# balkce/beamform

Hardware: AMD Instinct MI355X
Metric: stft_frames_per_sec (higher is better)
Workload: dtype f64; 1 GPU; das 8-mic 1024-pt (hop 512), 65536-frame batch per GPU, 1 stream(s), planar input resident in HBM; frames_per_gpu=65536, frames_fed_per_gpu=65536, mics=8, fft=1024, hop=512, streams=1, layout=planar, gather=n/a, parallelism=independent batches x1, input=uniform noise in [-0.5, 0.5), settle_launches_before_warmup=408, forward_transforms_per_frame_pair=6

## Files before the change

### beamform_amd/csrc/das_f64_plan.hpp

```cpp
#pragma once

#include <cstdlib>
#include <cstring>

#if defined(__HIPCC__)
#define BF_PLAN_HD __host__ __device__ inline
#else
#define BF_PLAN_HD inline
#endif

namespace bf {

constexpr int kChunkEnd = 0xFFFFF;
constexpr int kMaxChunkPairs = 1000;
constexpr int kSchedMaxChunks = 16384;

struct DasSchedPlan {
    int n_levels;
    int cnt[8], size[8];
    int n_chunks;
    int grid;
};

BF_PLAN_HD void das_f64_chunk(const DasSchedPlan &p, long n_frames, int n_streams, int k, int *stream, long *t0, long *n) {
    int lvl = 0, kk = k;
    long pair0 = 0;
    while (lvl < p.n_levels - 1 && kk >= p.cnt[lvl] * n_streams) {
        kk -= p.cnt[lvl] * n_streams;
        pair0 += (long)p.cnt[lvl] * p.size[lvl];
        ++lvl;
    }
    const int s = kk / p.cnt[lvl], j = kk - s * p.cnt[lvl];
    *stream = s;
    *t0 = 2 * (pair0 + (long)j * p.size[lvl]);
    long len = 2L * p.size[lvl];
    if (*t0 + len > n_frames) len = n_frames - *t0;
    *n = len;
}

inline DasSchedPlan das_f64_plan(long n_frames, int n_streams, int n_cus, const char *env) {
    DasSchedPlan p{};
    const long pairs = (n_frames + 1) / 2;
    long nb = (long)n_cus / n_streams;
    if (nb < 1) nb = 1;
    int sizes[8], n_sizes = 0;
    const long share = (pairs + nb - 1) / nb;
    if (env && strchr(env, ',')) {
        const char *c = env;
        while (*c && n_sizes < 8) {
            sizes[n_sizes++] = atoi(c);
            c = strchr(c, ',');
            if (!c) break;
            ++c;
        }
    } else if (!(env && atoi(env) == 0) && share >= 48) {
        long front = (share * 13 / 16) & ~7L;
        long rest = share - front;
        while (front > kMaxChunkPairs && n_sizes < 3) {
            sizes[n_sizes++] = kMaxChunkPairs;
            front -= kMaxChunkPairs;
        }
        if (front > kMaxChunkPairs) { rest += front - kMaxChunkPairs; front = kMaxChunkPairs; }
        sizes[n_sizes++] = (int)front;
        while (n_sizes < 6 && rest >= 24) {
            long sz = (rest / 2) & ~7L;
            if (sz > kMaxChunkPairs) sz = kMaxChunkPairs;
            sizes[n_sizes++] = (int)sz;
            rest -= sz;
        }
        if (rest >= 12) { sizes[n_sizes++] = 4; rest -= 4; }
        sizes[n_sizes++] = 2;
// ... 33 lines not shown
```

### beamform_amd/csrc/das_f64_w64.hip

```cpp
#include <hip/hip_runtime.h>

#include <type_traits>

#include "launch_trace.hpp"
#include "pipeline_kernels.hpp"
#include "switches.hpp"
#include "w64_f64_dev.hpp"

namespace bf {

namespace {

constexpr int kBlock = 512;
constexpr int kWaves = kBlock / 64;
constexpr int kHop = 512;
constexpr int kTwD = 2 * (1024 + 4 * kTw2RowW64Rot);
constexpr int oTw = 0;
constexpr int oPlane = kTwD;
constexpr int oGain = oPlane + kWaves * kPlaneD;
constexpr int oCross = oGain + 4 * 2048;
constexpr int oFlag = oCross + 512;
constexpr int kWinRow = 18;
constexpr int oWin = oFlag + 8;
constexpr int kLdsD = oWin + 64 * kWinRow;
// ... 253 lines not shown
constexpr int kGMic = 8 * kGRow;
constexpr int kSlots = 64;
constexpr int kTwP = 2 * (960 + 4 * kTw2RowW64Rot);
constexpr int pTw = 0;
constexpr int pPlane = kTwP;
constexpr int pGain = pPlane + kWaves * kPlaneD;
constexpr int pFlag = pGain + 7 * kGMic * 2;
constexpr int kRingR = 32;
constexpr int kRingSlots = kRingR + kWaves;
constexpr int pRing = pFlag + (kSlots + 4) / 2;
constexpr int pWin = pRing + kRingR / 2;
constexpr int kLdsP = pWin + 64 * kWinRow;
static_assert(kLdsP * 8 <= 160 * 1024, "LDS");
static_assert((pGain & 1) == 0 && (pWin & 1) == 0, "16-byte alignment");


typedef volatile __attribute__((address_space(3))) int *lds_int_t;
typedef volatile __attribute__((address_space(3))) unsigned long long *lds_u64_t;
__device__ __forceinline__ int lds_fetch_add(lds_int_t p, int v, int lane) {
    int old = 0;
    if (lane == 0) old = __hip_atomic_fetch_add((__attribute__((address_space(3))) int *)p, v, __ATOMIC_RELAXED, __HIP_MEMORY_SCOPE_WORKGROUP);
    return __builtin_amdgcn_readfirstlane(old);
}
__device__ __forceinline__ unsigned long long lds_fetch_add64(lds_u64_t p, int lane) {
    unsigned long long old = 0;
    if (lane == 0) old = __hip_atomic_fetch_add((__attribute__((address_space(3))) unsigned long long *)p, 1ull, __ATOMIC_RELAXED, __HIP_MEMORY_SCOPE_WORKGROUP);
    const unsigned lo = (unsigned)__builtin_amdgcn_readfirstlane((int)(unsigned)old), hi = (unsigned)__builtin_amdgcn_readfirstlane((int)(unsigned)(old >> 32));
    return ((unsigned long long)hi << 32) | lo;
}
struct DasSched {
    const int4 *chunks;
    unsigned *counter;
    int n_chunks;
};
__device__ __forceinline__ unsigned long long pack_work(unsigned vbase, int chunk, int pairs, int next) {
    return ((unsigned long long)(vbase & 0xFFFFFFu) << 40) | ((unsigned long long)(unsigned)chunk << 20) | ((unsigned long long)(unsigned)pairs << 10) | (unsigned)next;
}
struct PairWork {
    int4 d;
    int pos;
    int len;
    unsigned u;
    bool have;
};
__device__ __forceinline__ int4 load_chunk(const int4 *chunks, int k) {
    const int4 d = chunks[k];
    return int4{__builtin_amdgcn_readfirstlane(d.x), __builtin_amdgcn_readfirstlane(d.y), __builtin_amdgcn_readfirstlane(d.z), k};
}
__device__ __forceinline__ PairWork draw_pair(lds_u64_t work, const DasSched &sc, int lane, const int4 held) {
    PairWork r;
    r.have = false;
    r.d = int4{0, 0, 0, 0};
    r.pos = r.len = 0;
    r.u = 0;
    for (;;) {
        const unsigned long long old = lds_fetch_add64(work, lane);
        const int pos = (int)(old & 1023u), len = (int)((old >> 10) & 1023u), k = (int)((old >> 20) & 0xFFFFFu);
        const unsigned vb = (unsigned)(old >> 40);
        if (k == kChunkEnd) return r;
        if (pos < len) {
            if (k == held.w) r.d = held;
            else r.d = load_chunk(sc.chunks, k);
            r.pos = pos; r.len = len; r.u = vb + (unsigned)pos; r.have = true;
            return r;
        }
        if (pos == len) {
            unsigned k2 = 0;
            if (lane == 0) k2 = __hip_atomic_fetch_add(sc.counter, 1u, __ATOMIC_RELAXED, __HIP_MEMORY_SCOPE_AGENT);
            k2 = (unsigned)__builtin_amdgcn_readfirstlane((int)k2);
            if (k2 >= (unsigned)sc.n_chunks) {
                if (lane == 0) *work = pack_work(vb + (unsigned)len, kChunkEnd, 0, 0);
                return r;
            }
            r.d = load_chunk(sc.chunks, (int)k2);
            r.len = (r.d.z + 1) >> 1;
            r.pos = 0; r.u = vb + (unsigned)len; r.have = true;
            if (lane == 0) *work = pack_work(r.u, (int)k2, r.len, 1);
            return r;
        }
        while ((int)((*work >> 20) & 0xFFFFFu) == k) __builtin_amdgcn_s_sleep(2);
    }
}
__device__ __forceinline__ int claim_boundary(lds_int_t st, unsigned b, int lane) {
    const int base = 4 * (int)(b / kSlots);
    while (st[b & (kSlots - 1)] < base) __builtin_amdgcn_s_sleep(1);
    return lds_fetch_add(st + (b & (kSlots - 1)), 1, lane) - base;
}
__device__ __forceinline__ void publish_boundary(lds_int_t st, unsigned b, int lane) { (void)lds_fetch_add(st + (b & (kSlots - 1)), 2, lane); }
__device__ __forceinline__ void skip_boundary(lds_int_t st, unsigned b, int lane) {
    const int base = 4 * (int)(b / kSlots);
    while (st[b & (kSlots - 1)] < base) __builtin_amdgcn_s_sleep(1);
    (void)lds_fetch_add(st + (b & (kSlots - 1)), 4, lane);
}
__device__ __forceinline__ void await_boundary(lds_int_t st, unsigned b) {
    while (st[b & (kSlots - 1)] - 4 * (int)(b / kSlots) < 3) __builtin_amdgcn_s_sleep(1);
}

#ifdef BF_W64_STATS
__device__ unsigned long long g_stats[256 * 8 * 5];
#define BF_STATS_DECL unsigned long long st_[5] = {0, 0, 0, 0, 0}; const unsigned long long st_t0_ = __builtin_amdgcn_s_memrealtime()
#define BF_STAT(i) (++st_[i])
#define BF_STAT_WAIT_BEGIN const unsigned long long st_w0_ = __builtin_amdgcn_s_memrealtime()
#define BF_STAT_WAIT_END st_[3] += __builtin_amdgcn_s_memrealtime() - st_w0_
#define BF_STATS_FLUSH do { st_[4] = __builtin_amdgcn_s_memrealtime() - st_t0_; if (lane == 0 && blockIdx.x < 256) for (int i_ = 0; i_ < 5; ++i_) g_stats[(blockIdx.x * 8 + w) * 5 + i_] = st_[i_]; } while (0)
#else
#define BF_STATS_DECL
#define BF_STAT(i) ((void)0)
#define BF_STAT_WAIT_BEGIN
#define BF_STAT_WAIT_END
#define BF_STATS_FLUSH
#endif
#ifdef BF_W64_STAMPS
__device__ unsigned long long g_stamps[256 * 8 * 64];
#define BF_STAMP(slot) do { if (lane == 0 && blockIdx.x < 256 && (slot) < 64) g_stamps[(blockIdx.x * 8 + w) * 64 + (slot)] = __builtin_amdgcn_s_memrealtime(); } while (0)
#else
// ... 160 lines not shown
        }
        __builtin_amdgcn_fence(__ATOMIC_ACQUIRE, "workgroup");
        return r;
    };
    auto release_pair = [&](const PairWork &pw, bool has_t) {
        const unsigned u2 = 2u * pw.u;
        (void)lds_fetch_add(s_ring + (u2 & (kRingR - 1)), 2, lane);
        (void)lds_fetch_add(s_ring + ((u2 + 1) & (kRingR - 1)), has_t ? 1 : 2, lane);
        if (pw.pos > 0) (void)lds_fetch_add(s_ring + ((u2 - 1) & (kRingR - 1)), 1, lane);
    };
    auto request_ring_mic = [&](const RingHops &r, int m) { request(r.h + m * kHop, r.a + m * kHop, r.b + m * kHop); };
    auto request_ring_extra = [&](bool on, const RingHops &r) {
        if (!on) {
#pragma unroll
            for (int j = 0; j < 8; ++j) e0[j] = e1[j] = e2[j] = 0.f;
            return;
        }
#pragma unroll
        for (int j = 0; j < 8; ++j) {
            e0[j] = r.h[XM * kHop + (unsigned)(64 * j + lane)];
            e1[j] = r.a[XM * kHop + (unsigned)(64 * j + lane)];
            e2[j] = r.b[XM * kHop + (unsigned)(64 * j + lane)];
        }
    };
    RingHops curR{nullptr, nullptr, nullptr};
    (void)curR;

    BF_STAMP(0);
#ifdef BF_W64_STAMPS
    if (lane == 0 && blockIdx.x < 256) g_stamps[(blockIdx.x * 8 + w) * 64 + 59] = __builtin_amdgcn_s_memtime();
#endif
    PairWork cur;
    cur.d = load_chunk(sc.chunks, (int)blockIdx.x);
    cur.len = (cur.d.z + 1) >> 1;
    const int n_static = cur.len < kWaves ? cur.len : kWaves;
    cur.pos = w;
    cur.u = (unsigned)w;
    cur.have = w < n_static;
    if (LAYOUT == 0 && cur.have) {
        request_pair_mic(cur.d.x, cur.d.y + 2L * w, a.slot_mic[0]);
        request_extra(XM >= 0, cur.d.x, cur.d.y + 2L * w);
    } else {
        request_extra(false, 0, 0);
    }
    {
        const f64x2 *tw2 = a.tw + 64;
        f64x2 *ltw = reinterpret_cast<f64x2 *>(lds + pTw), *lg = reinterpret_cast<f64x2 *>(lds + pGain);
#pragma unroll 4
        for (int i = tid; i < kTwP / 2; i += kBlock) ltw[i] = tw2[i];
        for (int k = 0; k < NT; ++k) {
            const f64x2 *g2 = a.gains_mic + a.slot_mic[k] * kGMic;
#pragma unroll 2
            for (int i = tid; i < kGMic; i += kBlock) lg[k * kGMic + i] = g2[i];
        }
#pragma unroll 2
        for (int i = tid; i < 1024; i += kBlock) lds[pWin + (i & 63) * kWinRow + (i >> 6)] = a.win[i];
        if (tid < kSlots) s_state[tid] = 0;
        if (tid < kRingR) s_ring[tid] = 0;
        if (tid == 0) *s_work = pack_work(0u, (int)blockIdx.x, cur.len, n_static);
    }
    __syncthreads();
    BF_STAMP(1);
    BF_STATS_DECL;
    int it = 0;
    if (!cur.have) {
        cur = draw_pair(s_work, sc, lane, cur.d);
        if (LAYOUT == 0 && cur.have) {
            request_pair_mic(cur.d.x, cur.d.y + 2L * cur.pos, a.slot_mic[0]);
            request_extra(XM >= 0, cur.d.x, cur.d.y + 2L * cur.pos);
        }
    }
    while (cur.have) {
        if constexpr (LAYOUT == 1) {
            curR = prepare_pair(cur);
            request_ring_mic(curR, a.slot_mic[0]);
            request_ring_extra(XM >= 0, curR);
        }
        const int stream = cur.d.x;
        const long T0 = cur.d.y, T1 = T0 + cur.d.z;
        const long tA = T0 + 2L * cur.pos;
        const bool pair = tA + 1 < T1;
        const long tL = pair ? tA + 1 : tA;
        const unsigned u = cur.u;
        const bool has_t = cur.pos + 1 < cur.len, has_h = cur.pos > 0;
        float *ys = a.y + (long)stream * a.n_frames * kHop;
        PairWork nxt;
        nxt.have = false;
        const float *hp0 = a.x + (long)stream * a.stream_stride_x + tA * kHop;
        const float *hist0 = a.hist + (long)stream * M * kHop;
        const bool first_hop = tA < 1, last_hop = !(tA + 1 < a.n_frames);
        (void)hp0; (void)hist0; (void)first_hop; (void)last_hop;

        double Sr[16], Si[16];
        auto one_mic = [&](const int k, auto first_tag) {
            constexpr bool FIRST = decltype(first_tag)::value;
            double re[16], im[16];
#ifndef BF_PAIR_NO_VMWAIT
            if constexpr (!FIRST) __builtin_amdgcn_s_waitcnt(0x0F70);
#endif
// ... 3 lines not shown
                    const double w0 = wrow[j], w1 = wrow[j + 8];
                    const double c = (double)n1[j] + (double)e1[j];
                    const double t = ((double)n0[j] + (double)e0[j]) * w0;
                    re[j] = fma(c, w1, t);
                    re[j + 8] = fma(-c, w1, t);
                    const double t2 = c * w0, u2 = (double)n2[j] + (double)e2[j];
                    im[j] = fma(u2, w1, t2);
                    im[j + 8] = fma(-u2, w1, t2);
                }
            } else {
#pragma unroll
                for (int j = 0; j < 8; ++j) {
                    const double w0 = wrow[j], w1 = wrow[j + 8];
                    const double c = (double)n1[j];
                    const double t = (double)n0[j] * w0;
                    re[j] = fma(c, w1, t);
                    re[j + 8] = fma(-c, w1, t);
                    const double t2 = c * w0, u2 = (double)n2[j];
                    im[j] = fma(u2, w1, t2);
                    im[j + 8] = fma(-u2, w1, t2);
                }
            }
            if (__builtin_expect(!pair, 0)) {
#ifndef BF_PAIR_CNDMASK
                asm volatile("" ::: "memory");
#endif
#pragma unroll
                for (int j = 0; j < 16; ++j) im[j] = 0.0;
            }
            if (k + 1 < NT) {
                if constexpr (LAYOUT == 1) request_ring_mic(curR, a.slot_mic[k + 1]);
                else request_pair_mic(stream, tA, a.slot_mic[k + 1]);
            } else {
                nxt = draw_pair(s_work, sc, lane, cur.d);
                if constexpr (LAYOUT == 0) {
                    if (nxt.have) request_pair_mic(nxt.d.x, nxt.d.y + 2L * nxt.pos, a.slot_mic[0]);
                    else request_pair_mic(stream, tA, a.slot_mic[0]);
                }
            }
            cx<double> tw[15];
            BF_STAGE();
            load_tw1<1, 9>(tw, s_tw1, lane);
            BF_STAGE();
            fft16_core<double, -1, true, 1>(re, im);
            BF_STAGE();
            load_tw1<9, 16>(tw, s_tw1, lane);
            BF_STAGE();
            mul_tw<false, 1, 9>(re, im, tw);
            BF_STAGE();
            mul_tw<false, 9, 16>(re, im, tw);
            BF_STAGE();
            T1_fwd(re, im, wcol, row16);
            load_tw2<1, 9>(tw, s_tw2, lane);
            BF_STAGE();
            fft16_core<double, -1, true>(re, im);
            BF_STAGE();
            load_tw2<9, 16>(tw, s_tw2, lane);
            BF_STAGE();
            mul_tw<false, 1, 9>(re, im, tw);
            BF_STAGE();
            mul_tw<false, 9, 16>(re, im, tw);
            BF_STAGE();
            w64_T2_any<true>(re, im, row16 - 16 * (lane >> 4), lane >> 4);
            cxa g[16];
            const lds_gain_t gd = (lds_gain_t)(size_t)(gd0 + (unsigned)(k * kGMic * 16));
            const lds_gain_t gm = (lds_gain_t)(size_t)((g_mirror + (unsigned)(2 * k * kGMic * 16)) - (gd0 + (unsigned)(k * kGMic * 16)));
            BF_STAGE();
// ... 82 lines not shown
            oT = claim_boundary(s_state, u, lane);
            if (oT == 0) {
#pragma unroll
                for (int j = 0; j < 8; ++j) yn[(unsigned)(64 * j + lane)] = tl[j];
            }
        } else {
            skip_boundary(s_state, u, lane);
        }
#pragma unroll
        for (int j = 0; j < 16; ++j) {
            const float f = (float)Sr[j];
            oA[j] = (float)((double)f * wrow[j]);
        }
        if (pair) {
            float *y1 = ys + (tA + 1) * kHop;
#pragma unroll
            for (int j = 0; j < 8; ++j) {
                const float f0 = (float)Si[j];
                const float b0 = (float)((double)f0 * wrow[j]);
                y1[(unsigned)(64 * j + lane)] = oA[j + 8] + b0;
            }
        }
        if (has_h) {
            oH = claim_boundary(s_state, u - 1, lane);
            if (oH == 0) {
#pragma unroll
                for (int j = 0; j < 8; ++j) yo[(unsigned)(64 * j + lane)] = oA[j];
            }
        } else if (T0 == 0) {
            const float *ti = a.tail_in + (long)stream * kHop;
#pragma unroll
            for (int j = 0; j < 8; ++j) yo[(unsigned)(64 * j + lane)] = ti[(unsigned)(64 * j + lane)] + oA[j];
        } else {
#pragma unroll
            for (int j = 0; j < 8; ++j) atomicAdd(yo + (unsigned)(64 * j + lane), oA[j]);
        }
        if (oT == 0 || oH == 0) {
            __builtin_amdgcn_fence(__ATOMIC_RELEASE, "workgroup");
            if (oT == 0) publish_boundary(s_state, u, lane);
            if (oH == 0) publish_boundary(s_state, u - 1, lane);
        }
        if (oT > 0) {
            BF_STAT(2);
            BF_STAT_WAIT_BEGIN;
            await_boundary(s_state, u);
            BF_STAT_WAIT_END;
            __builtin_amdgcn_fence(__ATOMIC_ACQUIRE, "workgroup");
            float o[8];
#pragma unroll
            for (int j = 0; j < 8; ++j) o[j] = BF_PARK_LD(yn + (unsigned)(64 * j + lane));
#pragma unroll
            for (int j = 0; j < 8; ++j) yn[(unsigned)(64 * j + lane)] = tl[j] + o[j];
        } else {
            BF_STAT(0);
        }
        if (oH > 0) {
            BF_STAT(2);
            BF_STAT_WAIT_BEGIN;
            await_boundary(s_state, u - 1);
            BF_STAT_WAIT_END;
            __builtin_amdgcn_fence(__ATOMIC_ACQUIRE, "workgroup");
            float o[8];
#pragma unroll
            for (int j = 0; j < 8; ++j) o[j] = BF_PARK_LD(yo + (unsigned)(64 * j + lane));
#pragma unroll
            for (int j = 0; j < 8; ++j) yo[(unsigned)(64 * j + lane)] = o[j] + oA[j];
        } else {
            BF_STAT(1);
        }
        if (!has_t) {
            if (T1 < a.n_frames) {
                float *ynx = ys + T1 * kHop;
#pragma unroll
                for (int j = 0; j < 8; ++j) atomicAdd(ynx + (unsigned)(64 * j + lane), tl[j]);
            } else {
                float *to = a.tail_out + (long)stream * kHop;
#pragma unroll
                for (int j = 0; j < 8; ++j) to[(unsigned)(64 * j + lane)] = tl[j];
                if (a.hist_out != nullptr) {
                    float *ho = a.hist_out + (long)stream * M * kHop;
                    const float *xs = a.x + (long)stream * a.stream_stride_x;
                    for (int m = 0; m < M; ++m) {
                        const float *xl = xs + (long)m * a.mic_stride + tL * kHop;
#pragma unroll
                        for (int j = 0; j < 8; ++j) ho[m * kHop + 64 * j + lane] = xl[(unsigned)(64 * j + lane)];
                    }
                }
            }
        }
        if constexpr (LAYOUT == 1) {
            asm volatile("" ::: "memory");
            release_pair(cur, has_t);
        }
        cur = nxt;
        ++it;
    }
    BF_STATS_FLUSH;
#ifdef BF_W64_STAMPS
    if (lane == 0 && blockIdx.x < 256) {
        g_stamps[(blockIdx.x * 8 + w) * 64 + 63] = __builtin_amdgcn_s_memrealtime();
        g_stamps[(blockIdx.x * 8 + w) * 64 + 60] = __builtin_amdgcn_s_memtime();
        g_stamps[(blockIdx.x * 8 + w) * 64 + 62] = (unsigned long long)it;
        g_stamps[(blockIdx.x * 8 + w) * 64 + 61] = (unsigned long long)__builtin_amdgcn_s_getreg(((4 - 1) << 11) | (0 << 6) | 20);
    }
#endif
    (void)it;
}

__global__ __launch_bounds__(kBlock) void das_f64_pair_kernel(DasF64Args a, DasSched sc) { das_f64_pair_body<0>(a, sc); }
__global__ __launch_bounds__(kBlock) void das_f64_ring_kernel(DasF64Args a, DasSched sc) { das_f64_pair_body<1>(a, sc); }

constexpr int kSchedPerBlock = 8;
__global__ __launch_bounds__(32 * kSchedPerBlock) void das_f64_sched_kernel(DasSchedPlan p, int4 *chunks, unsigned *counter, float *y, long n_frames, int n_streams) {
    const int k = blockIdx.x * kSchedPerBlock + (int)(threadIdx.x >> 5), l = (int)(threadIdx.x & 31);
    if (k >= p.n_chunks) return;
    int stream;
    long t0, n;
    das_f64_chunk(p, n_frames, n_streams, k, &stream, &t0, &n);
    if (l == 0) {
        chunks[k] = int4{stream, (int)t0, (int)n, 0};
        if (k == 0) *counter = (unsigned)p.grid;
    }
    if (t0 > 0) {
        float4 *h = reinterpret_cast<float4 *>(y + ((long)stream * n_frames + t0) * kHop);
        for (int i = l; i < kHop / 4; i += 32) h[i] = float4{0.f, 0.f, 0.f, 0.f};
    }
}

__global__ __launch_bounds__(256) void interleaved_to_planar_kernel(const float *x, float *out, long tiles_per_stream, int M, long in_stream_stride,
                                                                    long out_mic_stride, long out_stream_stride) {
    __shared__ float s_t[256 * 9];
    const int tid = threadIdx.x;
    const long s = blockIdx.x / tiles_per_stream, tile = blockIdx.x - s * tiles_per_stream;
    const float4 *src = reinterpret_cast<const float4 *>(x + s * in_stream_stride + tile * 256 * M);
    const int R = M + 1;
    for (int i = tid; i < 64 * M; i += 256) {
        const float4 v = src[i];
        const int e = 4 * i;
        s_t[(e / M) * R + e % M] = v.x;
        s_t[((e + 1) / M) * R + (e + 1) % M] = v.y;
        s_t[((e + 2) / M) * R + (e + 2) % M] = v.z;
        s_t[((e + 3) / M) * R + (e + 3) % M] = v.w;
    }
    __syncthreads();
    float *dst = out + s * out_stream_stride + tile * 256;
    for (int j = tid; j < 64 * M; j += 256) {
        const int m = j >> 6, q = j & 63;
        const float4 v{s_t[(4 * q) * R + m], s_t[(4 * q + 1) * R + m], s_t[(4 * q + 2) * R + m], s_t[(4 * q + 3) * R + m]};
        reinterpret_cast<float4 *>(dst + (long)m * out_mic_stride)[q] = v;
    }
}

}

constexpr size_t kSchedCounterBytes = 256;
size_t das_f64_sched_ws_bytes() { return kSchedCounterBytes + (size_t)kSchedMaxChunks * sizeof(int4); }

DasF64Launch das_f64_decide(int layout, int n_mics, int n_streams, long n_frames, int n_cus, bool mic0_unit, int n_tr, bool tables) {
    DasF64Launch d{};
    if (n_mics > 8) return d;
    const bool ring = switches().das_il_ring != 0 && (n_mics == 2 || n_mics == 4 || n_mics == 8);
    bool frame_pair = tables && mic0_unit && n_mics >= 2 && n_tr >= 1;
    if (layout != BF_PLANAR && !ring && ((n_frames * kHop) & 255) != 0) frame_pair = false;
    if (!frame_pair) {
        if (layout == BF_PLANAR) return d;
        const long runs = n_cus > n_streams ? n_cus / n_streams : 1;
        d.path = DasF64Path::kMicPair;
        d.run_frames = ((n_frames + runs - 1) / runs + kWaves - 1) / kWaves * kWaves;
        d.runs_per_stream = (n_frames + d.run_frames - 1) / d.run_frames;
        return d;
    }
    if ((long)n_streams * ((n_frames + 1) / 2) >= (1L << 31)) return d;
    d.plan = das_f64_plan(n_frames, n_streams, n_cus, switches().das_f64_sched);
    if (d.plan.n_chunks < 1 || d.plan.n_chunks > kSchedMaxChunks) return d;
    d.path = layout == BF_PLANAR ? DasF64Path::kFramePair : ring ? DasF64Path::kRing : DasF64Path::kTranspose;
    d.writes_hist = layout == BF_PLANAR;
    const size_t hop_elems = (size_t)n_mics * kHop;
    d.scratch_bytes = sizeof(float) * (layout == BF_PLANAR ? 0 : ring ? n_cus * kRingSlots * hop_elems : n_streams * hop_elems * (n_frames + 1));
    return d;
}

static hipError_t launch_interleaved_to_planar(const float *x, float *out, long n, int n_mics, int n_streams, hipStream_t s) {
    const long tiles = n / 256;
    BF_LAUNCH(interleaved_to_planar_kernel, dim3((unsigned)(tiles * n_streams)), dim3(256), 0, s, x, out, tiles, n_mics, (long)n_mics * n, n, (long)n_mics * n);
    return hipGetLastError();
}

hipError_t enqueue_das_f64(DasF64Args a, const DasF64Launch &d, float *scratch, hipStream_t s, hipEvent_t kev0, hipEvent_t kev1, bool *kev_recorded) {
    hipError_t e = hipSuccess;
    int4 *const chunks = reinterpret_cast<int4 *>(reinterpret_cast<char *>(a.sched_ws) + kSchedCounterBytes);
    const DasSched sc{chunks, reinterpret_cast<unsigned *>(a.sched_ws), d.plan.n_chunks};
    if (d.path == DasF64Path::kMicPair) {
        for (int st = 0; st < a.n_streams && d.runs_per_stream > 1; ++st) {
            e = hipMemset2DAsync(a.y + ((long)st * a.n_frames + d.run_frames) * kHop, (size_t)d.run_frames * kHop * sizeof(float), 0, kHop * sizeof(float), (size_t)d.runs_per_stream - 1, s);
            if (e != hipSuccess) return e;
        }
    } else {
        if (d.path == DasF64Path::kRing) {
            a.ring = scratch; a.ring_bytes = d.scratch_bytes; a.hist_out = nullptr;
        } else if (d.path == DasF64Path::kTranspose) {
            const long n = a.n_frames * kHop;
            float *const hist = scratch + (size_t)a.n_streams * a.n_mics * n;
            if ((e = launch_interleaved_to_planar(a.x, scratch, n, a.n_mics, a.n_streams, s)) != hipSuccess) return e;
            if ((e = launch_interleaved_to_planar(a.hist, hist, kHop, a.n_mics, a.n_streams, s)) != hipSuccess) return e;
            a.x = scratch; a.hist = hist; a.hist_out = nullptr; a.mic_stride = n; a.layout = BF_PLANAR;
        }
        BF_LAUNCH(das_f64_sched_kernel, dim3((unsigned)((sc.n_chunks + kSchedPerBlock - 1) / kSchedPerBlock)), dim3(32 * kSchedPerBlock), 0, s, d.plan, chunks, sc.counter, a.y, a.n_frames, a.n_streams);
        if ((e = hipGetLastError()) != hipSuccess) return e;
    }
    if (kev0 && (e = hipEventRecord(kev0, s)) != hipSuccess) return e;
    if (d.path == DasF64Path::kMicPair)
        BF_LAUNCH(das_f64_w64_kernel<1>, dim3((unsigned)(d.runs_per_stream * a.n_streams)), dim3(kBlock), 0, s, a, (int)d.run_frames, (int)d.runs_per_stream);
    else if (d.path == DasF64Path::kRing)
        BF_LAUNCH(das_f64_ring_kernel, dim3((unsigned)d.plan.grid), dim3(kBlock), 0, s, a, sc);
    else
        BF_LAUNCH(das_f64_pair_kernel, dim3((unsigned)d.plan.grid), dim3(kBlock), 0, s, a, sc);
    if ((e = hipGetLastError()) != hipSuccess) return e;
    if (kev1 && (e = hipEventRecord(kev1, s)) == hipSuccess) *kev_recorded = true;
    return e;
}

}

#ifdef BF_W64_STATS
extern "C" int bf_dbg_stats(unsigned long long *host) {
    return (int)hipMemcpyFromSymbol(host, HIP_SYMBOL(bf::g_stats), sizeof(unsigned long long) * 256 * 8 * 5);
}
#endif
#ifdef BF_W64_STAMPS
extern "C" int bf_dbg_stamps(unsigned long long *host) {
    return (int)hipMemcpyFromSymbol(host, HIP_SYMBOL(bf::g_stamps), sizeof(unsigned long long) * 256 * 8 * 64);
}
#endif
```

### beamform_amd/csrc/pipeline.hip

```cpp
#include "pipeline.hpp"

#include <hip/hip_runtime.h>

#include <cmath>
#include <vector>

#include "device_mem.hpp"
#include "fft1024.hpp"
#include "pipeline_kernels.hpp"
#include "switches.hpp"

namespace bf {

namespace {

class BinPipelineImpl : public Engine {
    static constexpr int kMaxCols = BF_MAX_INTERF + 1;
   public:
    BinPipelineImpl(const bf_config &c, int n_cus) : cfg_(c), n_cus_(n_cus) {
        M_ = c.n_mics;
        H_ = c.hop;
        N_ = 2 * c.hop;
        NQ_ = problems_per_frame(N_);
        YS_ = yh_stride(N_);
// ... 26 lines not shown
        }
        if (cov_node_ && (Phist_ < 1 || Phist_ > 64)) {
            err_ = "past_windows must be in 1..64";
            return BF_EINVAL;
        }
        if (time_node_ && (M_ > 16 || cfg_.gsc_filter_size < 1 || cfg_.gsc_filter_size > 256)) {
            err_ = "gsc is built for up to 16 microphones and filter_size 1..256";
            return M_ > 16 ? BF_ENOSYS : BF_EINVAL;
        }
        if (cfg_.algo == BF_PHASEMPF && (cfg_.smooth_size < 1 || cfg_.smooth_size > 64)) {
            err_ = "smooth_size must be in 1..64";
            return BF_EINVAL;
        }
        ENGINE_HIP(d_tw_.upload(N_ == 1024 ? twiddle_table_32x32<f64x2>() : stockham_twiddles<f64x2>(N_)));
        ENGINE_HIP(d_tw32_.upload(twiddle_table_32x32<f32x2>()));
        ENGINE_HIP(d_win_.upload(sqrt_hann(N_)));
        freqs_ = frequency_vector(N_, cfg_.sample_rate);
        ENGINE_HIP(d_freq_.upload(freqs_));
        skip_lo_ = N_; band_yh_hi_ = NQ_ - 1;
        if (band_node_) {
            int klo = N_, khi = 0;
            for (int q = 1; q < NQ_; ++q) {
                const double f = std::fabs(freqs_[q]);
                if (f >= cfg_.freq_min && f <= cfg_.freq_max) { if (q < klo) klo = q; khi = q; }
            }
            if (khi < N_ / 2 - 2) { skip_lo_ = khi; skip_hi_ = N_ - khi; }
            if (cov_node_ && khi < N_ / 2 - 1 && klo <= khi) { band_yh_lo_ = klo; band_yh_hi_ = khi; }
            else if (cov_node_ && klo > khi) { band_yh_lo_ = 1; band_yh_hi_ = 0; }
        }
        for (auto &b : d_steer_) ENGINE_HIP(b.alloc(steer_elems()));
        if (das_one_launch_shape()) {
            for (auto &b : d_dasg_w64_) ENGINE_HIP(b.alloc((size_t)4 * 1024));
            for (auto &b : d_dasg_mic_) ENGINE_HIP(b.alloc((size_t)8 * kDasMicGainRows * kDasMicGainRow));
            ENGINE_HIP(d_das_sched_.alloc(das_f64_sched_ws_bytes()));
        }
        if (N_ == 1024) ENGINE_HIP(d_tw_w64_.upload(twiddle_table_w64_rot()));
        for (auto &b : d_hist2_) ENGINE_HIP(b.alloc(hist_elems()));
        for (auto &b : d_tail_) ENGINE_HIP(b.alloc(tail_elems()));
        if (Phist_ > 0) ENGINE_HIP(d_zhist_.alloc(zhist_bytes()));
        if (cfg_.algo == BF_GSS) {
            ENGINE_HIP(d_gssW_.alloc(gss_bytes() / sizeof(f64x2)));
            ENGINE_HIP(hipMemset(d_gssW_.get(), 0, gss_bytes()));
        }
        if (cfg_.algo == BF_PHASEMPF || cfg_.algo == BF_MCRA) ENGINE_HIP(d_mpf_.alloc(mpf_bytes() / sizeof(double)));
        if (cfg_.algo == BF_PHASEMPF) ENGINE_HIP(d_smooth_.alloc(smooth_bytes() / sizeof(double)));
        if (time_node_) ENGINE_HIP(d_nlms_.alloc(nlms_bytes() / sizeof(float)));
        return BF_OK;
    }

    int reset(hipStream_t st) override {
        ENGINE_HIP(hipMemsetAsync(d_hist2_[0].get(), 0, hist_elems() * sizeof(float), st));
        hist_cur_ = 0;
        for (auto &b : d_tail_) ENGINE_HIP(hipMemsetAsync(b.get(), 0, tail_elems() * sizeof(float), st));
        tail_cur_ = 0;
        if (d_zhist_.get()) ENGINE_HIP(hipMemsetAsync(d_zhist_.get(), 0, zhist_bytes(), st));
        if (d_mpf_.get()) ENGINE_HIP(hipMemsetAsync(d_mpf_.get(), 0, mpf_bytes(), st));
        if (d_smooth_.get()) ENGINE_HIP(hipMemsetAsync(d_smooth_.get(), 0, smooth_bytes(), st));
        if (d_nlms_.get()) ENGINE_HIP(hipMemsetAsync(d_nlms_.get(), 0, nlms_bytes(), st));
        gss_reset_mask_ = ~0ull;
        return BF_OK;
    }

    int upload_steering(const std::vector<SteeringSet> &dirs, hipStream_t stream) override {
        const int nc = dirs[0].n_cols, nd = (int)dirs.size();
        if ((size_t)nd * nc * M_ * N_ > steer_elems()) {
            err_ = "steering table larger than the device buffer";
            return BF_EINVAL;
        }
        std::vector<f64x2> t((size_t)nd * N_ * M_ * nc);
        for (int d = 0; d < nd; ++d)
            for (int c = 0; c < nc; ++c)
                for (int m = 0; m < M_; ++m)
                    for (int j = 0; j < N_; ++j) {
                        const cplxd w = dirs[d].at(j, m, c);
                        t[(((size_t)d * nc + c) * M_ + m) * N_ + j] = f64x2{w.real(), w.imag()};
                    }
        const int nxt = steer_cur_ ^ 1;
        std::vector<f64x2> dg, dg64, dgm;
        if (das_one_launch_shape()) {
            dg = das_pair_gains_t<f64x2>(dirs[0], 4);
            dg64 = das_pair_gains_w64_f64(dg, 4);
            ENGINE_HIP(hipMemcpyAsync(d_dasg_w64_[nxt].get(), dg64.data(), dg64.size() * sizeof(f64x2), hipMemcpyHostToDevice, stream));
            dgm = das_mic_gains_w64_f64(dirs[0], 8);
            ENGINE_HIP(hipMemcpyAsync(d_dasg_mic_[nxt].get(), dgm.data(), dgm.size() * sizeof(f64x2), hipMemcpyHostToDevice, stream));
            bool unit = true;
            for (int j = 0; j < N_ && unit; ++j) unit = dirs[0].at(j, 0, 0) == cplxd(1.0, 0.0);
            das_mic0_unit_[nxt] = unit;
// ... 79 lines not shown
        for (auto &s : segs) {
            if (!s.n) continue;
            if (to_host)
                ENGINE_HIP(hipMemcpy(p, s.d, s.n, hipMemcpyDeviceToHost));
            else
                ENGINE_HIP(hipMemcpy(s.d, p, s.n, hipMemcpyHostToDevice));
            p += s.n;
        }
        return BF_OK;
    }

    bf_config cfg_;
    int n_cus_, M_, MF_, NP_, S_, D_, So_, KP1_, Phist_;
    const bool cov_node_ = cfg_.algo == BF_MVDR || cfg_.algo == BF_LCMV;
    const bool band_node_ = cov_node_ || cfg_.algo == BF_GSS;
    const bool time_node_ = cfg_.algo == BF_GSC;
    const bool single_ch_ = cfg_.algo == BF_MCRA;
    const bool post_amp_ = band_node_;
    const bool yraw_target_ = cfg_.algo == BF_PHASEMPF || time_node_;
    int skip_lo_, skip_hi_ = 0;
    int band_yh_lo_ = 0, band_yh_hi_;
    bool z48_ = false;
    size_t zsz_ = sizeof(f64x2);
    int H_ = 512, N_ = 1024, NQ_ = 514, YS_ = 516;
    const KernelSet *ks_ = nullptr;
    long steer_dir_stride_ = 0;
    std::vector<double> freqs_;
    DeviceBuffer<f64x2> d_tw_;
    DeviceBuffer<f32x2> d_tw32_;
    DeviceBuffer<double> d_win_, d_freq_;
    DeviceBuffer<f64x2> d_steer_[2];
    DeviceBuffer<f64x2> d_dasg_w64_[2];
    DeviceBuffer<f64x2> d_tw_w64_;
    DeviceBuffer<char> d_das_sched_;
    DeviceBuffer<f64x2> d_dasg_mic_[2];
    bool das_mic0_unit_[2] = {false, false};
    DasSlots das_slots_[2];
    int steer_cur_ = 0;
    DeviceBuffer<float> d_hist2_[2];
    int hist_cur_ = 0;
    DeviceBuffer<float> d_tail_[2];
    int tail_cur_ = 0;
    DeviceBuffer<char> d_zhist_;
    DeviceBuffer<f64x2> d_gssW_;
    DeviceBuffer<double> d_mpf_;
    DeviceBuffer<double> d_smooth_;
    DeviceBuffer<float> d_nlms_;
    unsigned long long gss_reset_mask_ = ~0ull;
    DeviceBuffer<char> d_Z_;
    DeviceBuffer<char> d_Yh_;
    DeviceBuffer<float> d_yraw_;
    DeviceBuffer<float> d_planar_;
    DeviceBuffer<float> d_frames_;
};

int BinPipelineImpl::run_das_one_launch(const float *x, long F, float *y, hipStream_t stream, int layout, long mic_stride, const RunSnapshot &snap) {
    if (!das_one_launch_shape() || switches().fused_bins != 1 || snap.das_gains_w64 == nullptr) return kDeclined;
    const DasF64Launch d = das_f64_decide(layout, M_, S_, F, n_cus_, snap.das_mic0_unit, snap.das_slots.n_tr,
                                          snap.das_gains_mic != nullptr && d_das_sched_.get() != nullptr);
    if (d.path == DasF64Path::kChain) return kDeclined;
    ENGINE_HIP(d_planar_.reserve((d.scratch_bytes + sizeof(float) - 1) / sizeof(float)));
    float *const hist = d_hist2_[hist_cur_].get();
    DasF64Args da;
    da.x = x; da.hist = hist; da.hist_out = d_hist2_[hist_cur_ ^ 1].get(); da.y = y;
    da.tail_in = d_tail_[tail_cur_].get(); da.tail_out = d_tail_[tail_cur_ ^ 1].get();
    da.win = d_win_.get(); da.n_frames = F; da.mic_stride = mic_stride;
    da.stream_stride_x = (long)M_ * F * H_; da.n_streams = S_; da.n_mics = M_; da.run_len = 1;
    da.layout = layout;
    da.gains = snap.das_gains_w64; da.gains_mic = snap.das_gains_mic; da.tw = d_tw_w64_.get();
    da.mic0_unit = snap.das_mic0_unit ? 1 : 0;
    da.n_tr = snap.das_slots.n_tr; da.extra_mic = snap.das_slots.extra_mic;
    for (int k = 0; k < 8; ++k) da.slot_mic[k] = snap.das_slots.slot_mic[k];
    da.sched_ws = d_das_sched_.get(); da.sched_ws_bytes = d_das_sched_.get() ? das_f64_sched_ws_bytes() : 0;
    ENGINE_HIP(enqueue_das_f64(da, d, d_planar_.get(), stream, kev0, kev1, &kev_recorded));
    if (d.writes_hist)
        hist_cur_ ^= 1;
    else
        ENGINE_HIP(carry_last_hop(hist, x, F, H_, M_, S_, layout, mic_stride, (long)F * H_ * M_, stream));
    tail_cur_ ^= 1;
    return BF_OK;
}

int BinPipelineImpl::run(const float *x, long F, float *y, f64x2 *spectrum, hipStream_t stream, int layout, long mic_stride,
                         const RunSnapshot &snap) {
    const int rc = spectrum ? kDeclined : run_das_one_launch(x, F, y, stream, layout, mic_stride, snap);
    return rc == kDeclined ? run_chain(x, F, y, spectrum, stream, layout, mic_stride, snap) : rc;
}

int BinPipelineImpl::run_chain(const float *x, long F, float *y, f64x2 *spectrum, hipStream_t stream, int layout, long mic_stride,
                               const RunSnapshot &snap) {
    float *const hist = d_hist2_[hist_cur_].get();
    const long FT = Phist_ + F;
    const bool try_fused = switches().fused_bins != 0 && Phist_ == 0 && N_ <= 2048 && M_ <= 8 && MF_ == M_ && D_ == 1 &&
                           (cfg_.algo == BF_DAS || cfg_.algo == BF_PHASE || cfg_.algo == BF_PHASEMPF);
    if (!try_fused)
        ENGINE_HIP(d_Z_.reserve(((size_t)S_ * FT + (cov_node_ ? 512 : 0)) * NP_ * N_ * zsz_));
    else
        ENGINE_HIP(d_Z_.reserve((size_t)S_ * F * 2 * 8 * sizeof(f64x2)));
    ENGINE_HIP(d_Yh_.reserve((size_t)So_ * F * YS_ * (sizeof(f64x2) + (cfg_.algo == BF_PHASEMPF ? sizeof(double) : 0))));
    if (yraw_target_) ENGINE_HIP(d_yraw_.reserve((size_t)So_ * F * H_));
    if (N_ != 1024) ENGINE_HIP(d_frames_.reserve((size_t)So_ * F * N_));
    f64x2 *Z = (f64x2 *)d_Z_.get();
    f64x2 *const Yh = (f64x2 *)d_Yh_.get();
    const size_t frame_elems = (size_t)NP_ * N_;

    if (Phist_ > 0)
// ... 91 lines not shown
```

### beamform_amd/csrc/pipeline_kernels.hpp

```cpp
#pragma once

#include <hip/hip_runtime.h>

#include "../../include/bfcore.h"
#include "das_f64_plan.hpp"
#include "geometry.hpp"

namespace bf {

#ifdef BF_NFFT
#define BF_CAT2_(a, b) a##b
#define BF_CAT2(a, b) BF_CAT2_(a, b)
#define BF_NTAG BF_CAT2(n, BF_NFFT)
#endif

constexpr int problems_per_frame(int nfft) { return nfft / 2 + 2; }
constexpr int yh_stride(int nfft) { return nfft / 2 + 4; }
constexpr int kMpfVecs = 7;
#ifdef BF_NFFT
namespace BF_NTAG {
constexpr int kN = BF_NFFT;
constexpr int kHop = kN / 2;
constexpr int kNQ = problems_per_frame(kN);
constexpr int kYhStride = yh_stride(kN);
constexpr int kQX = kN / 2 + 1;
}
#endif

struct z48 {
    unsigned lo, re_hi, im_hi;
};

struct StftArgs {
    const float *x;
    const float *hist;
    f64x2 *Z;
    const f64x2 *tw;
    const double *win;
// ... 19 lines not shown
    int n_streams, n_mics, kp1;
    int n_dirs;
    long steer_dir_stride;
    bf_config cfg;
    f64x2 *gssW;
    double *mpf;
    unsigned long long gss_reset_mask;
    int z48;
    int rec_istft = 0;
    float *rec_y = nullptr;
    const float *rec_tail_in = nullptr;
    float *rec_tail_out = nullptr;
    const f64x2 *rec_tw_w64 = nullptr;
    const double *rec_win = nullptr;
    int mpf32;
};
struct IstftArgs {
    const f64x2 *Yh;
    int yh32;
    int yh_lo, yh_hi;
    float *y;
    const float *tail_in;
    float *tail_out;
    const f64x2 *tw;
    const f32x2 *tw32;
    const f64x2 *tw_w64 = nullptr;
    float *frames;
    const double *win;
    long n_frames;
    int n_streams;
    double post_amp;
    int use_post_amp;
};
struct DasF64Args {
    const float *x;
    const float *hist;
    float *y;
    const float *tail_in;
    float *tail_out;
    const f64x2 *gains;
    const f64x2 *tw;
    const double *win;
    long n_frames, mic_stride, stream_stride_x;
    int n_streams, n_mics, run_len;
    int layout = 0;
    float *hist_out = nullptr;
    const f64x2 *gains_mic = nullptr;
    int n_tr = 0, extra_mic = -1;
    int slot_mic[8] = {1, 2, 3, 4, 5, 6, 7, 0};
    int mic0_unit = 0;
    void *sched_ws = nullptr;
    size_t sched_ws_bytes = 0;
    float *ring = nullptr;
    size_t ring_bytes = 0;
};

enum class DasF64Path {
    kChain,
    kFramePair,
    kRing,
    kTranspose,
    kMicPair,
};
struct DasF64Launch {
    DasF64Path path;
    DasSchedPlan plan;
    long run_frames, runs_per_stream;
    size_t scratch_bytes;
    bool writes_hist;
};
DasF64Launch das_f64_decide(int layout, int n_mics, int n_streams, long n_frames, int n_cus, bool mic0_unit, int n_tr, bool tables);
hipError_t enqueue_das_f64(DasF64Args a, const DasF64Launch &d, float *scratch, hipStream_t s, hipEvent_t kev0, hipEvent_t kev1, bool *kev_recorded);
size_t das_f64_sched_ws_bytes();

#ifdef BF_NFFT
namespace BF_NTAG {
hipError_t launch_stft(const StftArgs &a, int n_cus, hipStream_t s);
hipError_t launch_bins(const BinsArgs &a, int n_cus, hipStream_t s);
hipError_t launch_stft_bins_fused(const StftArgs &a, const BinsArgs &b, int n_cus, hipStream_t s);
hipError_t launch_pointwise(const BinsArgs &a, hipStream_t s);
hipError_t launch_phasempf(const BinsArgs &a, int n_cus, hipStream_t s);
hipError_t launch_mcra_node(const BinsArgs &a, hipStream_t s);
hipError_t launch_mvdr_lcmv(const BinsArgs &a, int n_cus, hipStream_t s);
hipError_t launch_gss(const BinsArgs &a, int n_cus, hipStream_t s);
hipError_t launch_gsc_align(const BinsArgs &a, hipStream_t s);
hipError_t launch_expand_spectrum(const f64x2 *Yh, f64x2 *spectrum, long frames, hipStream_t s);
hipError_t launch_istft(const IstftArgs &a, int n_cus, hipStream_t s);
hipError_t launch_gsc_nlms(const float *aligned, float *y, float *state, long n_samples, int n_streams, int n_mics,
                           const bf_config &cfg, hipStream_t s);
hipError_t launch_smooth(const float *yraw, float *y, double *state, long n_frames, int n_streams, int smooth_size,
                         hipStream_t s);
}
#endif

struct KernelSet {
    int nfft;
    hipError_t (*stft)(const StftArgs &, int, hipStream_t);
    hipError_t (*bins)(const BinsArgs &, int, hipStream_t);
    hipError_t (*stft_bins)(const StftArgs &, const BinsArgs &, int, hipStream_t);
    hipError_t (*istft)(const IstftArgs &, int, hipStream_t);
    hipError_t (*smooth)(const float *, float *, double *, long, int, int, hipStream_t);
    hipError_t (*gsc_nlms)(const float *, float *, float *, long, int, int, const bf_config &, hipStream_t);
};
const KernelSet *kernel_set_n128();
const KernelSet *kernel_set_n256();
const KernelSet *kernel_set_n512();
// ... 19 lines not shown
```

Measured before the change: 135.8 million frames/s.

## Cache DAS chunk table on host and exchange chunk-edge halves without atomics

The per-call scheduler kernel is removed. It used to build the chunk table, reset the work counter and zero the boundary output hops. Now the chunk table is built on the host and uploaded only when the plan changes, and the work counter keeps running across calls from a host-tracked base. Chunk-boundary overlap-add no longer does float atomicAdd into zeroed output. Each side writes its half into a scratch buffer and bumps a per-boundary flag, and whichever side arrives second sums both halves and writes the hop. This removes a launch and its memset traffic per call, at the cost of extra scratch writes, a release/acquire fence and a pinned-host table cache.

Result: slower. 112.9 million frames/s (-16.9%).

```diff
diff --git a/beamform_amd/csrc/das_f64_plan.hpp b/beamform_amd/csrc/das_f64_plan.hpp
--- a/beamform_amd/csrc/das_f64_plan.hpp
+++ b/beamform_amd/csrc/das_f64_plan.hpp
@@ -37,6 +37,39 @@
     if (*t0 + len > n_frames) len = n_frames - *t0;
     *n = len;
 }
+
+struct DasChunkRow {
+    int stream, t0, n, rank;
+};
+static_assert(sizeof(DasChunkRow) == 16, "one 16-byte load per row");
+
+inline bool das_f64_same_plan(const DasSchedPlan &a, const DasSchedPlan &b) {
+    if (a.n_levels != b.n_levels || a.n_chunks != b.n_chunks || a.grid != b.grid) return false;
+    for (int i = 0; i < a.n_levels; ++i)
+        if (a.cnt[i] != b.cnt[i] || a.size[i] != b.size[i]) return false;
+    return true;
+}
+inline int das_f64_chunks_per_stream(const DasSchedPlan &p) {
+    int c = 0;
+    for (int i = 0; i < p.n_levels; ++i) c += p.cnt[i];
+    return c;
+}
+inline void das_f64_fill_table(const DasSchedPlan &p, long n_frames, int n_streams, DasChunkRow *rows) {
+    int k = 0, before = 0;
+    for (int lvl = 0; lvl < p.n_levels; ++lvl) {
+        for (int s = 0; s < n_streams; ++s)
+            for (int j = 0; j < p.cnt[lvl]; ++j, ++k) {
+                int stream;
+                long t0, n;
+                das_f64_chunk(p, n_frames, n_streams, k, &stream, &t0, &n);
+                rows[k] = DasChunkRow{stream, (int)t0, (int)n, before + j};
+            }
+        before += p.cnt[lvl];
+    }
+}
+BF_PLAN_HD int das_f64_boundary(int stream, int rank, int cps) { return stream * cps + rank; }
+BF_PLAN_HD unsigned das_f64_take(unsigned old, unsigned base, unsigned grid) { return grid + (old - base); }
+inline unsigned das_f64_next_base(unsigned base, const DasSchedPlan &p) { return base + (unsigned)p.n_chunks; }
 
 inline DasSchedPlan das_f64_plan(long n_frames, int n_streams, int n_cus, const char *env) {
     DasSchedPlan p{};
diff --git a/beamform_amd/csrc/das_f64_w64.hip b/beamform_amd/csrc/das_f64_w64.hip
--- a/beamform_amd/csrc/das_f64_w64.hip
+++ b/beamform_amd/csrc/das_f64_w64.hip
@@ -309,12 +309,17 @@
     const int4 *chunks;
     unsigned *counter;
     int n_chunks;
+    unsigned base, grid;
+    int cps;
+    int *state;
+    float *halves;
 };
 __device__ __forceinline__ unsigned long long pack_work(unsigned vbase, int chunk, int pairs, int next) {
     return ((unsigned long long)(vbase & 0xFFFFFFu) << 40) | ((unsigned long long)(unsigned)chunk << 20) | ((unsigned long long)(unsigned)pairs << 10) | (unsigned)next;
 }
 struct PairWork {
     int4 d;
+    int k;
     int pos;
     int len;
     unsigned u;
@@ -322,12 +327,13 @@
 };
 __device__ __forceinline__ int4 load_chunk(const int4 *chunks, int k) {
     const int4 d = chunks[k];
-    return int4{__builtin_amdgcn_readfirstlane(d.x), __builtin_amdgcn_readfirstlane(d.y), __builtin_amdgcn_readfirstlane(d.z), k};
-}
-__device__ __forceinline__ PairWork draw_pair(lds_u64_t work, const DasSched &sc, int lane, const int4 held) {
+    return int4{__builtin_amdgcn_readfirstlane(d.x), __builtin_amdgcn_readfirstlane(d.y), __builtin_amdgcn_readfirstlane(d.z), __builtin_amdgcn_readfirstlane(d.w)};
+}
+__device__ __forceinline__ PairWork draw_pair(lds_u64_t work, const DasSched &sc, int lane, const int4 held, const int held_k) {
     PairWork r;
     r.have = false;
     r.d = int4{0, 0, 0, 0};
+    r.k = 0;
     r.pos = r.len = 0;
     r.u = 0;
     for (;;) {
@@ -336,20 +342,22 @@
         const unsigned vb = (unsigned)(old >> 40);
         if (k == kChunkEnd) return r;
         if (pos < len) {
-            if (k == held.w) r.d = held;
+            if (k == held_k) r.d = held;
             else r.d = load_chunk(sc.chunks, k);
+            r.k = k;
             r.pos = pos; r.len = len; r.u = vb + (unsigned)pos; r.have = true;
             return r;
         }
         if (pos == len) {
             unsigned k2 = 0;
             if (lane == 0) k2 = __hip_atomic_fetch_add(sc.counter, 1u, __ATOMIC_RELAXED, __HIP_MEMORY_SCOPE_AGENT);
-            k2 = (unsigned)__builtin_amdgcn_readfirstlane((int)k2);
+            k2 = das_f64_take((unsigned)__builtin_amdgcn_readfirstlane((int)k2), sc.base, sc.grid);
             if (k2 >= (unsigned)sc.n_chunks) {
                 if (lane == 0) *work = pack_work(vb + (unsigned)len, kChunkEnd, 0, 0);
                 return r;
             }
             r.d = load_chunk(sc.chunks, (int)k2);
+            r.k = (int)k2;
             r.len = (r.d.z + 1) >> 1;
             r.pos = 0; r.u = vb + (unsigned)len; r.have = true;
             if (lane == 0) *work = pack_work(r.u, (int)k2, r.len, 1);
@@ -358,6 +366,31 @@
         while ((int)((*work >> 20) & 0xFFFFFu) == k) __builtin_amdgcn_s_sleep(2);
     }
 }
+__device__ __forceinline__ void chunk_edge(const DasSched &sc, int b, int side, const float (&mine)[8], float *hop, int lane) {
+    float *slot = sc.halves + ((size_t)b * 2 + (size_t)side) * kHop;
+#ifdef BF_EDGE_WT
+#pragma unroll
+    for (int j = 0; j < 8; ++j) __hip_atomic_store(slot + (unsigned)(64 * j + lane), mine[j], __ATOMIC_RELAXED, __HIP_MEMORY_SCOPE_AGENT);
+#else
+#pragma unroll
+    for (int j = 0; j < 8; ++j) slot[(unsigned)(64 * j + lane)] = mine[j];
+    __builtin_amdgcn_fence(__ATOMIC_RELEASE, "agent");
+#endif
+    asm volatile("s_waitcnt vmcnt(0)" ::: "memory");
+    int old = 0;
+    if (lane == 0) old = __hip_atomic_fetch_add(sc.state + b, 1, __ATOMIC_RELAXED, __HIP_MEMORY_SCOPE_AGENT);
+    old = __builtin_amdgcn_readfirstlane(old);
+    if (old & 1) {
+        __builtin_amdgcn_fence(__ATOMIC_ACQUIRE, "agent");
+        const float *other = sc.halves + ((size_t)b * 2 + (size_t)(side ^ 1)) * kHop;
+        float o[8];
+#pragma unroll
+        for (int j = 0; j < 8; ++j) o[j] = other[(unsigned)(64 * j + lane)];
+#pragma unroll
+        for (int j = 0; j < 8; ++j) hop[(unsigned)(64 * j + lane)] = o[j] + mine[j];
+    }
+}
+
 __device__ __forceinline__ int claim_boundary(lds_int_t st, unsigned b, int lane) {
     const int base = 4 * (int)(b / kSlots);
     while (st[b & (kSlots - 1)] < base) __builtin_amdgcn_s_sleep(1);
@@ -584,6 +617,7 @@
 #endif
     PairWork cur;
     cur.d = load_chunk(sc.chunks, (int)blockIdx.x);
+    cur.k = (int)blockIdx.x;
     cur.len = (cur.d.z + 1) >> 1;
     const int n_static = cur.len < kWaves ? cur.len : kWaves;
     cur.pos = w;
@@ -616,7 +650,7 @@
     BF_STATS_DECL;
     int it = 0;
     if (!cur.have) {
-        cur = draw_pair(s_work, sc, lane, cur.d);
+        cur = draw_pair(s_work, sc, lane, cur.d, cur.k);
         if (LAYOUT == 0 && cur.have) {
             request_pair_mic(cur.d.x, cur.d.y + 2L * cur.pos, a.slot_mic[0]);
             request_extra(XM >= 0, cur.d.x, cur.d.y + 2L * cur.pos);
@@ -686,7 +720,7 @@
                 if constexpr (LAYOUT == 1) request_ring_mic(curR, a.slot_mic[k + 1]);
                 else request_pair_mic(stream, tA, a.slot_mic[k + 1]);
             } else {
-                nxt = draw_pair(s_work, sc, lane, cur.d);
+                nxt = draw_pair(s_work, sc, lane, cur.d, cur.k);
                 if constexpr (LAYOUT == 0) {
                     if (nxt.have) request_pair_mic(nxt.d.x, nxt.d.y + 2L * nxt.pos, a.slot_mic[0]);
                     else request_pair_mic(stream, tA, a.slot_mic[0]);
@@ -835,8 +869,10 @@
 #pragma unroll
             for (int j = 0; j < 8; ++j) yo[(unsigned)(64 * j + lane)] = ti[(unsigned)(64 * j + lane)] + oA[j];
         } else {
-#pragma unroll
-            for (int j = 0; j < 8; ++j) atomicAdd(yo + (unsigned)(64 * j + lane), oA[j]);
+            float hd[8];
+#pragma unroll
+            for (int j = 0; j < 8; ++j) hd[j] = oA[j];
+            chunk_edge(sc, das_f64_boundary(stream, cur.d.w, sc.cps), 1, hd, yo, lane);
         }
         if (oT == 0 || oH == 0) {
             __builtin_amdgcn_fence(__ATOMIC_RELEASE, "workgroup");
@@ -873,9 +909,7 @@
         }
         if (!has_t) {
             if (T1 < a.n_frames) {
-                float *ynx = ys + T1 * kHop;
-#pragma unroll
-                for (int j = 0; j < 8; ++j) atomicAdd(ynx + (unsigned)(64 * j + lane), tl[j]);
+                chunk_edge(sc, das_f64_boundary(stream, cur.d.w + 1, sc.cps), 0, tl, ys + T1 * kHop, lane);
             } else {
                 float *to = a.tail_out + (long)stream * kHop;
 #pragma unroll
@@ -912,23 +946,6 @@
 
 __global__ __launch_bounds__(kBlock) void das_f64_pair_kernel(DasF64Args a, DasSched sc) { das_f64_pair_body<0>(a, sc); }
 __global__ __launch_bounds__(kBlock) void das_f64_ring_kernel(DasF64Args a, DasSched sc) { das_f64_pair_body<1>(a, sc); }
-
-constexpr int kSchedPerBlock = 8;
-__global__ __launch_bounds__(32 * kSchedPerBlock) void das_f64_sched_kernel(DasSchedPlan p, int4 *chunks, unsigned *counter, float *y, long n_frames, int n_streams) {
-    const int k = blockIdx.x * kSchedPerBlock + (int)(threadIdx.x >> 5), l = (int)(threadIdx.x & 31);
-    if (k >= p.n_chunks) return;
-    int stream;
-    long t0, n;
-    das_f64_chunk(p, n_frames, n_streams, k, &stream, &t0, &n);
-    if (l == 0) {
-        chunks[k] = int4{stream, (int)t0, (int)n, 0};
-        if (k == 0) *counter = (unsigned)p.grid;
-    }
-    if (t0 > 0) {
-        float4 *h = reinterpret_cast<float4 *>(y + ((long)stream * n_frames + t0) * kHop);
-        for (int i = l; i < kHop / 4; i += 32) h[i] = float4{0.f, 0.f, 0.f, 0.f};
-    }
-}
 
 __global__ __launch_bounds__(256) void interleaved_to_planar_kernel(const float *x, float *out, long tiles_per_stream, int M, long in_stream_stride,
                                                                     long out_mic_stride, long out_stream_stride) {
@@ -956,8 +973,18 @@
 
 }
 
-constexpr size_t kSchedCounterBytes = 256;
-size_t das_f64_sched_ws_bytes() { return kSchedCounterBytes + (size_t)kSchedMaxChunks * sizeof(int4); }
+static hipError_t das_f64_queue_prepare(DasF64Queue &q, const DasSchedPlan &plan, long n_frames, int n_streams, hipStream_t s) {
+    hipError_t e;
+    if ((e = q.halves.reserve((size_t)plan.n_chunks * 2 * kHop)) != hipSuccess) return e;
+    if (q.n_frames == n_frames && q.n_streams == n_streams && das_f64_same_plan(q.plan, plan)) return hipSuccess;
+    if ((e = hipEventSynchronize(q.uploaded)) != hipSuccess) return e;
+    das_f64_fill_table(plan, n_frames, n_streams, q.host_rows.get());
+    q.n_frames = -1;
+    if ((e = hipMemcpyAsync(q.table.get(), q.host_rows.get(), (size_t)plan.n_chunks * sizeof(DasChunkRow), hipMemcpyHostToDevice, s)) != hipSuccess) return e;
+    if ((e = hipEventRecord(q.uploaded, s)) != hipSuccess) return e;
+    q.plan = plan; q.n_frames = n_frames; q.n_streams = n_streams;
+    return hipSuccess;
+}
 
 DasF64Launch das_f64_decide(int layout, int n_mics, int n_streams, long n_frames, int n_cus, bool mic0_unit, int n_tr, bool tables) {
     DasF64Launch d{};
@@ -991,8 +1018,7 @@
 
 hipError_t enqueue_das_f64(DasF64Args a, const DasF64Launch &d, float *scratch, hipStream_t s, hipEvent_t kev0, hipEvent_t kev1, bool *kev_recorded) {
     hipError_t e = hipSuccess;
-    int4 *const chunks = reinterpret_cast<int4 *>(reinterpret_cast<char *>(a.sched_ws) + kSchedCounterBytes);
-    const DasSched sc{chunks, reinterpret_cast<unsigned *>(a.sched_ws), d.plan.n_chunks};
+    DasSched sc{};
     if (d.path == DasF64Path::kMicPair) {
         for (int st = 0; st < a.n_streams && d.runs_per_stream > 1; ++st) {
             e = hipMemset2DAsync(a.y + ((long)st * a.n_frames + d.run_frames) * kHop, (size_t)d.run_frames * kHop * sizeof(float), 0, kHop * sizeof(float), (size_t)d.runs_per_stream - 1, s);
@@ -1008,8 +1034,16 @@
             if ((e = launch_interleaved_to_planar(a.hist, hist, kHop, a.n_mics, a.n_streams, s)) != hipSuccess) return e;
             a.x = scratch; a.hist = hist; a.hist_out = nullptr; a.mic_stride = n; a.layout = BF_PLANAR;
         }
-        BF_LAUNCH(das_f64_sched_kernel, dim3((unsigned)((sc.n_chunks + kSchedPerBlock - 1) / kSchedPerBlock)), dim3(32 * kSchedPerBlock), 0, s, d.plan, chunks, sc.counter, a.y, a.n_frames, a.n_streams);
-        if ((e = hipGetLastError()) != hipSuccess) return e;
+        DasF64Queue &q = *a.queue;
+        if ((e = das_f64_queue_prepare(q, d.plan, a.n_frames, a.n_streams, s)) != hipSuccess) return e;
+        char *const ws = q.ctl.get();
+        sc.chunks = reinterpret_cast<const int4 *>(q.table.get());
+        sc.counter = reinterpret_cast<unsigned *>(ws);
+        sc.n_chunks = d.plan.n_chunks;
+        sc.base = q.counter_base; sc.grid = (unsigned)d.plan.grid;
+        sc.cps = das_f64_chunks_per_stream(d.plan);
+        sc.state = reinterpret_cast<int *>(ws + DasF64Queue::kCounterBytes);
+        sc.halves = q.halves.get();
     }
     if (kev0 && (e = hipEventRecord(kev0, s)) != hipSuccess) return e;
     if (d.path == DasF64Path::kMicPair)
@@ -1019,6 +1053,7 @@
     else
         BF_LAUNCH(das_f64_pair_kernel, dim3((unsigned)d.plan.grid), dim3(kBlock), 0, s, a, sc);
     if ((e = hipGetLastError()) != hipSuccess) return e;
+    if (d.path != DasF64Path::kMicPair) a.queue->counter_base = das_f64_next_base(a.queue->counter_base, d.plan);
     if (kev1 && (e = hipEventRecord(kev1, s)) == hipSuccess) *kev_recorded = true;
     return e;
 }
diff --git a/beamform_amd/csrc/pipeline.hip b/beamform_amd/csrc/pipeline.hip
--- a/beamform_amd/csrc/pipeline.hip
+++ b/beamform_amd/csrc/pipeline.hip
@@ -82,7 +82,7 @@
         if (das_one_launch_shape()) {
             for (auto &b : d_dasg_w64_) ENGINE_HIP(b.alloc((size_t)4 * 1024));
             for (auto &b : d_dasg_mic_) ENGINE_HIP(b.alloc((size_t)8 * kDasMicGainRows * kDasMicGainRow));
-            ENGINE_HIP(d_das_sched_.alloc(das_f64_sched_ws_bytes()));
+            ENGINE_HIP(das_queue_.init());
         }
         if (N_ == 1024) ENGINE_HIP(d_tw_w64_.upload(twiddle_table_w64_rot()));
         for (auto &b : d_hist2_) ENGINE_HIP(b.alloc(hist_elems()));
@@ -103,6 +103,7 @@
         hist_cur_ = 0;
         for (auto &b : d_tail_) ENGINE_HIP(hipMemsetAsync(b.get(), 0, tail_elems() * sizeof(float), st));
         tail_cur_ = 0;
+        ENGINE_HIP(das_queue_.reset(st));
         if (d_zhist_.get()) ENGINE_HIP(hipMemsetAsync(d_zhist_.get(), 0, zhist_bytes(), st));
         if (d_mpf_.get()) ENGINE_HIP(hipMemsetAsync(d_mpf_.get(), 0, mpf_bytes(), st));
         if (d_smooth_.get()) ENGINE_HIP(hipMemsetAsync(d_smooth_.get(), 0, smooth_bytes(), st));
@@ -248,7 +249,7 @@
     DeviceBuffer<f64x2> d_steer_[2];
     DeviceBuffer<f64x2> d_dasg_w64_[2];
     DeviceBuffer<f64x2> d_tw_w64_;
-    DeviceBuffer<char> d_das_sched_;
+    DasF64Queue das_queue_;
     DeviceBuffer<f64x2> d_dasg_mic_[2];
     bool das_mic0_unit_[2] = {false, false};
     DasSlots das_slots_[2];
@@ -273,7 +274,7 @@
 int BinPipelineImpl::run_das_one_launch(const float *x, long F, float *y, hipStream_t stream, int layout, long mic_stride, const RunSnapshot &snap) {
     if (!das_one_launch_shape() || switches().fused_bins != 1 || snap.das_gains_w64 == nullptr) return kDeclined;
     const DasF64Launch d = das_f64_decide(layout, M_, S_, F, n_cus_, snap.das_mic0_unit, snap.das_slots.n_tr,
-                                          snap.das_gains_mic != nullptr && d_das_sched_.get() != nullptr);
+                                          snap.das_gains_mic != nullptr && das_queue_.ready());
     if (d.path == DasF64Path::kChain) return kDeclined;
     ENGINE_HIP(d_planar_.reserve((d.scratch_bytes + sizeof(float) - 1) / sizeof(float)));
     float *const hist = d_hist2_[hist_cur_].get();
@@ -287,7 +288,7 @@
     da.mic0_unit = snap.das_mic0_unit ? 1 : 0;
     da.n_tr = snap.das_slots.n_tr; da.extra_mic = snap.das_slots.extra_mic;
     for (int k = 0; k < 8; ++k) da.slot_mic[k] = snap.das_slots.slot_mic[k];
-    da.sched_ws = d_das_sched_.get(); da.sched_ws_bytes = d_das_sched_.get() ? das_f64_sched_ws_bytes() : 0;
+    da.queue = &das_queue_;
     ENGINE_HIP(enqueue_das_f64(da, d, d_planar_.get(), stream, kev0, kev1, &kev_recorded));
     if (d.writes_hist)
         hist_cur_ ^= 1;
diff --git a/beamform_amd/csrc/pipeline_kernels.hpp b/beamform_amd/csrc/pipeline_kernels.hpp
--- a/beamform_amd/csrc/pipeline_kernels.hpp
+++ b/beamform_amd/csrc/pipeline_kernels.hpp
@@ -4,6 +4,7 @@
 
 #include "../../include/bfcore.h"
 #include "das_f64_plan.hpp"
+#include "device_mem.hpp"
 #include "geometry.hpp"
 
 namespace bf {
@@ -89,6 +90,41 @@
     double post_amp;
     int use_post_amp;
 };
+struct DasF64Queue {
+    static constexpr size_t kCounterBytes = 256;
+    static constexpr size_t kCtlBytes = kCounterBytes + (size_t)kSchedMaxChunks * sizeof(int);
+    DeviceBuffer<char> ctl;
+    DeviceBuffer<DasChunkRow> table;
+    DeviceBuffer<float> halves;
+    PinnedBuffer<DasChunkRow> host_rows;
+    hipEvent_t uploaded = nullptr;
+    DasSchedPlan plan{};
+    long n_frames = -1;
+    int n_streams = 0;
+    unsigned counter_base = 0;
+    DasF64Queue() = default;
+    DasF64Queue(const DasF64Queue &) = delete;
+    DasF64Queue &operator=(const DasF64Queue &) = delete;
+    ~DasF64Queue() {
+        if (uploaded) (void)hipEventDestroy(uploaded);
+    }
+    hipError_t init() {
+        hipError_t e;
+        if ((e = ctl.alloc(kCtlBytes)) != hipSuccess) return e;
+        if ((e = table.alloc(kSchedMaxChunks)) != hipSuccess) return e;
+        if ((e = host_rows.alloc(kSchedMaxChunks)) != hipSuccess) return e;
+        if (!uploaded && (e = hipEventCreateWithFlags(&uploaded, hipEventDisableTiming)) != hipSuccess) return e;
+        n_frames = -1;
+        counter_base = 0;
+        return hipMemset(ctl.get(), 0, kCtlBytes);
+    }
+    hipError_t reset(hipStream_t s) {
+        if (!ready()) return hipSuccess;
+        counter_base = 0;
+        return hipMemsetAsync(ctl.get(), 0, kCtlBytes, s);
+    }
+    bool ready() const { return ctl.get() != nullptr && table.get() != nullptr; }
+};
 struct DasF64Args {
     const float *x;
     const float *hist;
@@ -106,8 +142,7 @@
     int n_tr = 0, extra_mic = -1;
     int slot_mic[8] = {1, 2, 3, 4, 5, 6, 7, 0};
     int mic0_unit = 0;
-    void *sched_ws = nullptr;
-    size_t sched_ws_bytes = 0;
+    DasF64Queue *queue = nullptr;
     float *ring = nullptr;
     size_t ring_bytes = 0;
 };
@@ -128,7 +163,6 @@
 };
 DasF64Launch das_f64_decide(int layout, int n_mics, int n_streams, long n_frames, int n_cus, bool mic0_unit, int n_tr, bool tables);
 hipError_t enqueue_das_f64(DasF64Args a, const DasF64Launch &d, float *scratch, hipStream_t s, hipEvent_t kev0, hipEvent_t kev1, bool *kev_recorded);
-size_t das_f64_sched_ws_bytes();
 
 #ifdef BF_NFFT
 namespace BF_NTAG {
```
